# twosigma/Cook

Hardware: NVIDIA H100
Metric: job x offer fit evals/sec per scheduling cycle (higher is better)
Workload: dtype f64

## Files before the change

cook_b200/csrc/match.cu:

```cuda
#include <cooperative_groups.h>

#include <algorithm>
#include <mutex>
#include <numeric>

#include "fold.cuh"
#include "sort.cuh"

namespace {

constexpr int RES_THREADS = 512;
constexpr int TOPK = 8;
constexpr int ROW_V_OFF = TOPK * 32 * 8;
constexpr int ROW_BYTES = TOPK * 32 * (8 + 4);

struct __align__(32) VmStatic { double lc, lm, rc, rm; };
struct __align__(32) VmDyn { double ac, am, yc, ym; };
struct __align__(8) VmCnt { int an, pu; };

struct __align__(16) VmCons {
  int hostname_id, location, max_tasks, num_tasks;
  int run_count, flags, gpu_lo, ports_total;
  long long host_start;
  int disk_lo, disk_n;
// ... 514 lines not shown
              int tv = vv[i]; vv[i] = vv[i - 1]; vv[i - 1] = tv;
            }
          }
        }
      }
    }
  }
  const bool wany = __any_sync(0xffffffffu, f[0] > 0.0);
  if (wany) {
#pragma unroll
    for (int i = 0; i < TOPK; i++) { E.f[warp][i][lane] = f[i]; E.v[warp][i][lane] = vv[i]; }
  }
  if (lane == 0) E.any[warp] = wany ? 1 : 0;
  long long e1 = PROF ? clock64() : 0;
  __syncthreads();
  if (CONSTR && sparse)
    for (int wd = threadIdx.x; wd < a.sb_words; wd += NW * 32) __stcg(sbrow + wd, SP.sb[wd]);
  bool any = false;
#pragma unroll
  for (int w = 0; w < NW; w++) any |= E.any[w] != 0;
  if (any) {
    constexpr int PER = NW * TOPK / 32;
    static_assert(NW * TOPK % 32 == 0 && TOPK % PER == 0, "partial lists split evenly over the lanes");
#pragma unroll 1
    for (int ci = 0; ci < CPW; ci++) {
      const int c = warp + ci * NW;
      const int sw = lane / (TOPK / PER), so = (lane % (TOPK / PER)) * PER;
      double lf[PER];
      int lv[PER];
#pragma unroll
      for (int j = 0; j < PER; j++) {
        const bool has = E.any[sw] != 0;
        lf[j] = has ? E.f[sw][so + j][c] : 0.0;
        lv[j] = has ? E.v[sw][so + j][c] : 0x7fffffff;
      }
      double of = 0.0;
      int ov = -1;
#pragma unroll 1
      for (int i = 0; i < TOPK; i++) {
        unsigned wk;
        int wl;
        const double wf = warp_argmax(lf[0], (unsigned)lv[0], wk, wl);
        if (!(wf > 0.0)) break;
        if (lane == i) { of = wf; ov = (int)wk; }
        if (lane == wl) {
#pragma unroll
          for (int q = 0; q < PER - 1; q++) { lf[q] = lf[q + 1]; lv[q] = lv[q + 1]; }
          lf[PER - 1] = 0.0; lv[PER - 1] = 0x7fffffff;
        }
      }
      if (lane < TOPK) {
        __stcg(rf + lane * 32 + c, of);
        __stcg(rv + lane * 32 + c, ov);
      }
    }
  }
  long long e2 = PROF ? clock64() : 0;
  __syncthreads();
  if (threadIdx.x == 0) {
    if (any) atomicMax(a.feas + (size_t)(blk & 1) * a.bmax + ib, blk + 1);
    asm volatile("red.release.gpu.global.add.u32 [%0], %1;" ::"l"(a.rows_ready + blk), "r"(1u) : "memory");
  }
  if (PROF) {
    long long e3 = clock64();
    ep[0] += (unsigned long long)(e1 - e0); ep[1] += (unsigned long long)(e2 - e1);
    ep[2] += (unsigned long long)(e3 - e2);
  }
}

constexpr int MAXB = 512;
constexpr int LOGN = 2 * MAXB;
constexpr int RING = 32;
constexpr int GRING = 64;
constexpr int MAX_SPEC_CTAS = 8;
constexpr int KC = 16;
#ifndef COOK_LK
#define COOK_LK 4
#endif
constexpr int LK = COOK_LK;
#ifndef COOK_NCW
#define COOK_NCW 4
#endif
constexpr int NCW = COOK_NCW;

enum { Q_JOB = 0, Q_END = 1, Q_EXIT = 2 };

struct Latest {
  int* s;
  int* g;
  __device__ __forceinline__ int get(int v) const { return g ? g[v] : s[v]; }
  __device__ __forceinline__ void set(int v, int e) const { if (g) g[v] = e; else s[v] = e; }
};

__device__ __forceinline__ void fence_cta() { asm volatile("fence.acq_rel.cta;" ::: "memory"); }
__device__ __forceinline__ void compiler_barrier() { asm volatile("" ::: "memory"); }

struct QEntry {
  int type, blk, k, lo;
  double jc, jm, jg;
  int jports, jj, grp, row;
};

struct __align__(16) LogEnt {
  int vm, an, pu, k;
  double ac, am, lc, lm, rc, rm, yc, ym;
};

struct Cand {
  double f;
  VmState st;
  int vm, e;
};

struct __align__(16) SpecOut {
  int type, s, n, complete;
  double zf;
  int gver, pad;
  int zv, z_real;
  Cand c[KC + 1];
};

static_assert(sizeof(SpecOut) % 16 == 0, "candidate sets travel with cp.async.bulk (16 B granules)");
static_assert(RING == 32, "the fetcher warp owns one result slot per lane");

struct ResolverShared {
  LogEnt log[LOGN];
  int4 logx[LOGN];
  QEntry q[RING];
  SpecOut res[RING + 1];
  unsigned long long res_bar[RING];
  volatile int q_seq[RING];
  volatile unsigned long long chain;
  volatile int exit_g;
  int ticket;
  volatile int lo_ring[4];
  volatile int bk_ring[8];
  volatile int bk_known;
  volatile int out_done, blk_c0, last_b;
};

__device__ __forceinline__ int chain_gdone(unsigned long long w) { return (int)(w >> 32); }
__device__ __forceinline__ int chain_ncommit(unsigned long long w) { return (int)(unsigned)w; }
__device__ __forceinline__ unsigned long long chain_pack(int gdone, int ncommit) {
  return ((unsigned long long)(unsigned)gdone << 32) | (unsigned)ncommit;
}

template <bool CONSTR>
__device__ __forceinline__ VmState load_log(const ResolverShared& S, int idx, int& vm, int& k) {
  const LogEnt* e = &S.log[idx & (LOGN - 1)];
  const int4 h = *reinterpret_cast<const int4*>(e);
  const double2 a0 = *reinterpret_cast<const double2*>(&e->ac);
  const double2 a1 = *reinterpret_cast<const double2*>(&e->lc);
  const double2 a2 = *reinterpret_cast<const double2*>(&e->rc);
  const double2 a3 = *reinterpret_cast<const double2*>(&e->yc);
  VmState st;
  vm = h.x; st.an = h.y; st.pu = h.z; k = h.w;
  st.ac = a0.x; st.am = a0.y; st.lc = a1.x; st.lm = a1.y; st.rc = a2.x; st.rm = a2.y; st.yc = a3.x; st.ym = a3.y;
  st.room = 0x7fffffff; st.occ = 0; st.ptot = 0;
  if (CONSTR) {
    const int4 x = S.logx[idx & (LOGN - 1)];
    st.room = x.x; st.occ = x.y; st.ptot = x.z;
  }
  return st;
}
template <bool CONSTR>
__device__ __forceinline__ void store_log(ResolverShared& S, int idx, int vm, int k, const VmState& st) {
  LogEnt* e = &S.log[idx & (LOGN - 1)];
  *reinterpret_cast<int4*>(e) = make_int4(vm, st.an, st.pu, k);
  *reinterpret_cast<double2*>(&e->ac) = make_double2(st.ac, st.am);
  *reinterpret_cast<double2*>(&e->lc) = make_double2(st.lc, st.lm);
  *reinterpret_cast<double2*>(&e->rc) = make_double2(st.rc, st.rm);
  *reinterpret_cast<double2*>(&e->yc) = make_double2(st.yc, st.ym);
  if (CONSTR) S.logx[idx & (LOGN - 1)] = make_int4(st.room, st.occ, st.ptot, 0);
}

struct LaneList {
  double f[LK];
  int v[LK], e[LK];
  double cbf, dbf;
  int cbv, dbv;
  bool cb_real;
  __device__ __forceinline__ void init() {
#pragma unroll
    for (int i = 0; i < LK; i++) { f[i] = 0.0; v[i] = 0x7fffffff; e[i] = -1; }
    cbf = dbf = 0.0; cbv = dbv = 0x7fffffff; cb_real = false;
  }
  __device__ __forceinline__ void push_front(double x, int xv, int xe) {
#pragma unroll
    for (int i = LK - 1; i > 0; i--) { f[i] = f[i - 1]; v[i] = v[i - 1]; e[i] = e[i - 1]; }
    f[0] = x; v[0] = xv; e[0] = xe;
  }
  __device__ __forceinline__ void insert(double x, int xv, int xe) {
    if (!(x > 0.0)) return;
    if (!better(x, xv, f[LK - 1], v[LK - 1])) {
      if (better(x, xv, dbf, dbv)) { dbf = x; dbv = xv; }
      return;
    }
    if (f[LK - 1] > 0.0 && better(f[LK - 1], v[LK - 1], dbf, dbv)) { dbf = f[LK - 1]; dbv = v[LK - 1]; }
    f[LK - 1] = x; v[LK - 1] = xv; e[LK - 1] = xe;
#pragma unroll
    for (int i = LK - 1; i > 0; i--) {
      if (better(f[i], v[i], f[i - 1], v[i - 1])) {
        double tf = f[i]; f[i] = f[i - 1]; f[i - 1] = tf;
        int tv = v[i]; v[i] = v[i - 1]; v[i - 1] = tv;
        int te = e[i]; e[i] = e[i - 1]; e[i - 1] = te;
      }
    }
  }
};


__device__ __forceinline__ int group_version(const MatchArgs& a, int j) {
  int v = 0;
  for (int q = a.jb.group_off[j]; q < a.jb.group_off[j + 1]; q++) v += __ldcg(a.gr.gp_n + a.jb.group_idx[q]);
  return v;
}

template <bool CONSTR>
__device__ __forceinline__ void spec_job(const MatchArgs& a, ResolverShared& S, const Latest latest, const QEntry& qe,
                                         const int s, const int depth, const int exact_n, SpecOut& out) {
  const int lane = threadIdx.x & 31;
// ... 81 lines not shown
    int cnt = __popc(q);
    if (cnt > depth - n) {
      unsigned wk;
      int wl;
      warp_argmax(qual ? hf : 0.0, (unsigned)hv, wk, wl);
      q = 1u << wl;
      cnt = 1;
    }
    if ((q >> lane) & 1u) {
      store_cand(n + __popc(q & ((1u << lane) - 1u)), hf, hv, he);
      taken |= 1u << hj;
    }
    n += cnt;
  }
  double zf;
  int zv, z_real = 0;
  {
    double ef = 0.0;
    int ev = 0x7fffffff, ee = -1;
    bool head = false;
#pragma unroll
    for (int j = LK - 1; j >= 0; j--)
      if (L.f[j] > 0.0 && !((taken >> j) & 1u)) { ef = L.f[j]; ev = L.v[j]; ee = L.e[j]; head = true; }
    if (L.cbf > 0.0 && better(L.cbf, L.cbv, ef, ev)) { ef = L.cbf; ev = L.cbv; head = false; }
    if (L.dbf > 0.0 && better(L.dbf, L.dbv, ef, ev)) { ef = L.dbf; ev = L.dbv; head = false; }
    zf = warp_max_f64(ef);
    zv = (int)__reduce_min_sync(0xffffffffu, (ef == zf && zf > 0.0) ? (unsigned)ev : 0xffffffffu);
    if (!(zf > 0.0)) complete = 1;
    else {
      const unsigned hm = __ballot_sync(0xffffffffu, ef == zf && ev == zv);
      const unsigned rm = __ballot_sync(0xffffffffu, ef == zf && ev == zv && head);
      if (hm == rm && hm != 0u) {
        z_real = 1;
        if (lane == __ffs(rm) - 1) store_cand(KC, zf, zv, ee);
      }
    }
  }
  if (lane == 0) { out.type = Q_JOB; out.s = s; out.n = n; out.complete = complete; out.zf = zf; out.zv = zv; out.z_real = z_real; out.gver = gver; }
  __syncwarp();
}

template <bool CONSTR>
__device__ __noinline__ void spec_job_fallback(const MatchArgs& a, ResolverShared& S, const Latest latest,
                                               const QEntry& qe, const int s) {
  spec_job<CONSTR>(a, S, latest, qe, s, 1, 1, S.res[RING]);
}

template <bool CONSTR>
__device__ __noinline__ int resolve_group_job(const MatchArgs& a, ResolverShared& S, const Latest latest,
                                              const QEntry& qe, VmState& w) {
  const int lane = threadIdx.x & 31;
  JobRegs r;
  r.c = qe.jc; r.m = qe.jm; r.g = qe.jg; r.ports = qe.jports; r.j = qe.jj;
  const unsigned* sbrow = CONSTR ? a.sbits + ((size_t)(qe.blk & 1) * a.bmax + qe.row) * a.sb_words : nullptr;
  double cf = 0.0;
  int cv = 0x7fffffff;
  for (int v = lane; v < a.of.O; v += 32) {
    const int e = latest.get(v);
    VmState st;
    if (e >= qe.lo) { int vm, k; st = load_log<CONSTR>(S, e, vm, k); }
    else st = load_snap<CONSTR>(a, qe.blk, v);
    const double f = eval_res<CONSTR>(a, r, v, st, true, CONSTR ? sb_global(sbrow, v) : true);
    if (f > cf) { cf = f; cv = v; }
  }
  unsigned wk;
  int wl;
  const double wf = warp_argmax(cf, (unsigned)cv, wk, wl);
  if (!(wf > 0.0)) return -1;
  const int wv = (int)wk;
  const int we = latest.get(wv);
  if (we >= qe.lo) { int vm, k; w = load_log<CONSTR>(S, we, vm, k); }
  else w = load_snap<CONSTR>(a, qe.blk, wv);
  return wv;
}

template <bool CONSTR, bool REMOTE>
__device__ void driver_warp(const MatchArgs& a, ResolverShared& S) {
  const int lane = threadIdx.x & 31;
  int g = 0;
  unsigned long long skipped = 0;
  auto wait_slot = [&](int gi) {
    while (chain_gdone(S.chain) <= gi - a.lookahead) __nanosleep(a.poll_ns);
  };
  for (int b = 0;; b++) {
    int k0, k1;
    if (!REMOTE) {
      while (S.bk_known < b + 1) __nanosleep(20);
      k0 = S.bk_ring[b & 7];
      k1 = S.bk_ring[(b + 1) & 7];
    } else {
      if (b >= 2) {
        if (lane == 0) {
          while ((int)ld_relaxed_u32(a.published) < b - 1) __nanosleep(64);
          __threadfence();
        }
        __syncwarp();
      }
      k0 = __ldcg(a.bk0 + b);
      k1 = __ldcg(a.bk0 + b + 1);
    }
    if (k0 >= a.n_cons) break;
    const int nj = min(k1, a.n_cons) - k0;
    int dead = 0;
    if (lane == 0) {
      while (ld_acquire_u32(a.rows_ready + b) < (unsigned)nj) {
        const int db = (int)ld_relaxed_u32(reinterpret_cast<const unsigned*>(a.dead_blk));
        if (db != 0 && db - 1 <= b) { dead = 1; break; }
        __nanosleep(20);
      }
    }
    dead = __shfl_sync(0xffffffffu, dead, 0);
    if (dead) {
      if (!REMOTE && lane == 0) {
        skipped += (unsigned long long)(a.n_cons - k0);
        *a.dead_k0 = k0;
      }
      break;
    }
    const int lo = b == 0 ? 0 : (REMOTE ? __ldcg(a.lo_g + b - 1) : S.lo_ring[(b - 1) & 3]);
    const int32_t* feas = a.feas + (size_t)(b & 1) * a.bmax;
    int stamp[MAXB / 32];
#pragma unroll
    for (int t = 0; t < MAXB / 32; t++) stamp[t] = (t * 32 + lane) < nj ? __ldcg(feas + t * 32 + lane) : 0;
#pragma unroll
    for (int t = 0; t < MAXB / 32; t++) {
      const int base = t * 32;
      if (base >= nj) break;
      const int i = base + lane;
      const bool valid = i < nj;
      const bool fz = valid && stamp[t] == b + 1;
      if (!REMOTE && valid && !fz) { a.assign[k0 + i] = -1; a.fail[k0 + i] = COOK_FAIL_RESOURCES; }
      const unsigned mask = __ballot_sync(0xffffffffu, fz);
      skipped += __popc(__ballot_sync(0xffffffffu, valid && !fz));
      if (fz) {
        const int gi = g + __popc(mask & ((1u << lane) - 1u));
        const int k = k0 + i;
        QEntry q;
        q.type = Q_JOB; q.blk = b; q.k = k; q.lo = lo;
        q.jc = a.kc[k]; q.jm = a.km[k]; q.jj = a.cons[k];
        q.jg = CONSTR ? a.kg[k] : 0.0;
        q.jports = CONSTR ? a.kports[k] : 0;
        q.grp = CONSTR ? (a.kflags[k] & 1) : 0;
        q.row = i;
        wait_slot(gi);
        S.q[gi & (RING - 1)] = q;
        fence_cta();
        S.q_seq[gi & (RING - 1)] = gi + 1;
      }
      g += __popc(mask);
      __syncwarp();
    }
    if (lane == 0) {
      wait_slot(g);
      QEntry& q = S.q[g & (RING - 1)];
      q.type = Q_END; q.blk = b; q.k = -1; q.lo = lo; q.grp = 0;
      if (!REMOTE) S.res[g & (RING - 1)].type = Q_END;
      fence_cta();
      S.q_seq[g & (RING - 1)] = g + 1;
      if (!REMOTE) mbar_arrive(&S.res_bar[g & (RING - 1)]);
    }
    g++;
    __syncwarp();
  }
  if (lane == 0) {
    wait_slot(g);
    S.q[g & (RING - 1)].type = Q_EXIT;
    if (!REMOTE) S.res[g & (RING - 1)].type = Q_EXIT;
    fence_cta();
    S.q_seq[g & (RING - 1)] = g + 1;
    if (!REMOTE) mbar_arrive(&S.res_bar[g & (RING - 1)]);
    S.exit_g = g;
    if (!REMOTE) a.stats[6] = skipped;
  }
}

template <bool CONSTR>
__device__ void spec_warp(const MatchArgs& a, ResolverShared& S, const Latest latest, const int ci) {
  const int lane = threadIdx.x & 31;
  while (true) {
    int t = 0;
    if (lane == 0) t = atomicAdd(&S.ticket, 1);
    t = __shfl_sync(0xffffffffu, t, 0);
    const int g = t * a.n_spec + ci;
    const int slot = g & (RING - 1);
    bool quit = false;
    while (S.q_seq[slot] != g + 1) {
      const int xg = S.exit_g;
      if (xg >= 0 && g > xg) { quit = true; break; }
      __nanosleep(a.poll_ns);
    }
    if (quit) return;
    compiler_barrier();
    const QEntry qe = S.q[slot];
    if (qe.type == Q_EXIT) return;
    if (qe.type != Q_JOB) continue;
    const int s = chain_ncommit(S.chain);
    compiler_barrier();
    spec_job<CONSTR>(a, S, latest, qe, s, KC, 2, a.gres[g & (GRING - 1)]);
    __threadfence();
    __syncwarp();
    if (lane == 0) st_release_u32(a.gres_seq + (g & (GRING - 1)), (unsigned)(g + 1));
  }
}

template <bool CONSTR>
__device__ void publisher_warp(const MatchArgs& a, ResolverShared& S) {
  const int lane = threadIdx.x & 31;
  int p = 0;
  unsigned long long last = 0ull;
  while (true) {
    const unsigned long long w = S.chain;
    compiler_barrier();
    if (w != last) {
      const int c = chain_ncommit(w);
      for (int base = p; base < c; base += 6) {
        const int e = base + lane / 5, ch = lane % 5;
        if (lane < 30 && e < c) {
          const int4 v = reinterpret_cast<const int4*>(&S.log[e & (LOGN - 1)])[ch];
          __stcg(reinterpret_cast<int4*>(a.glog + (e & (LOGN - 1))) + ch, v);
        }
      }
      if (CONSTR)
        for (int e = p + lane; e < c; e += 32) __stcg(a.glogx + (e & (LOGN - 1)), S.logx[e & (LOGN - 1)]);
      __threadfence();
      __syncwarp();
      if (lane == 0) st_release_u64(a.gchain, w);
      p = c;
      last = w;
    } else {
      __nanosleep(40);
    }
    const int xg = S.exit_g;
    if (xg >= 0 && chain_gdone(last) >= xg) return;
  }
}

template <bool CONSTR>
__device__ void follower_warp(const MatchArgs& a, ResolverShared& S, const Latest latest) {
  const int lane = threadIdx.x & 31;
  int p = 0;
  unsigned long long last = 0ull;
  while (true) {
    unsigned long long w = 0ull;
    if (lane == 0) w = ld_relaxed_u64(a.gchain);
    w = __shfl_sync(0xffffffffu, w, 0);
    if (w != last) {
      __threadfence();
      const int c = chain_ncommit(w);
      for (int base = p; base < c; base += 6) {
        const int e = base + lane / 5, ch = lane % 5;
// ... 2 lines not shown
          reinterpret_cast<int4*>(&S.log[e & (LOGN - 1)])[ch] = v;
        }
      }
      if (CONSTR)
        for (int e = p + lane; e < c; e += 32) S.logx[e & (LOGN - 1)] = __ldcg(a.glogx + (e & (LOGN - 1)));
      __syncwarp();
      if (lane == 0) {
        for (int e = p; e < c; e++) latest.set(S.log[e & (LOGN - 1)].vm, e);
        fence_cta();
        S.chain = w;
      }
      __syncwarp();
      p = c;
      last = w;
    } else {
      __nanosleep(40);
    }
    const int xg = S.exit_g;
    if (xg >= 0 && chain_gdone(last) >= xg) return;
  }
}

__device__ void fetcher_warp(const MatchArgs& a, ResolverShared& S) {
  const int lane = threadIdx.x & 31;
  int g = lane;
  bool have_q = false, done = false;
  while (true) {
    if (!done && !have_q) {
      if (S.q_seq[lane] == g + 1) {
        compiler_barrier();
        const int type = S.q[lane].type;
        if (type == Q_JOB) have_q = true;
        else if (type == Q_EXIT) done = true;
        else g += RING;
      } else {
        const int xg = S.exit_g;
        if (xg >= 0 && g > xg) done = true;
      }
    }
    bool issued = false;
    if (!done && have_q) {
      const int gi = g & (GRING - 1);
      if (ld_relaxed_u32(a.gres_seq + gi) == (unsigned)(g + 1)) {
        __threadfence();
        fence_proxy_async_global();
        mbar_arrive_expect_tx(&S.res_bar[lane], (unsigned)sizeof(SpecOut));
        bulk_g2s(&S.res[lane], a.gres + gi, (unsigned)sizeof(SpecOut), &S.res_bar[lane]);
        have_q = false;
        g += RING;
        issued = true;
      }
    }
    if (__all_sync(0xffffffffu, done)) return;
    if (!__any_sync(0xffffffffu, issued)) __nanosleep(a.poll_ns);
  }
}

__device__ __forceinline__ double warp_argmax_fast(double f, int v, int& wv, int& wl) {
  const unsigned hi = (unsigned)__double2hiint(f);
  const unsigned mh = __reduce_max_sync(0xffffffffu, hi);
  unsigned cand = __ballot_sync(0xffffffffu, hi == mh);
  if (mh == 0u) { wv = 0x7fffffff; wl = 0; return 0.0; }
  if (__popc(cand) > 1) {
    const unsigned lo = hi == mh ? (unsigned)__double2loint(f) : 0u;
    const unsigned ml = __reduce_max_sync(0xffffffffu, lo);
    cand = __ballot_sync(0xffffffffu, hi == mh && lo == ml);
    if (__popc(cand) > 1) {
      const unsigned key = ((cand >> (threadIdx.x & 31)) & 1u) ? (unsigned)v : 0xffffffffu;
      const unsigned mk = __reduce_min_sync(0xffffffffu, key);
      cand = __ballot_sync(0xffffffffu, key == mk);
    }
  }
  wl = __ffs(cand) - 1;
  wv = __shfl_sync(0xffffffffu, v, wl);
  return __shfl_sync(0xffffffffu, f, wl);
}

template <bool CONSTR, bool PROF>
__device__ void commit_warp(const MatchArgs& a, ResolverShared& S, const Latest latest, const int cw,
                            unsigned* sbw) {
  const int lane = threadIdx.x & 31;
  unsigned long long n_fast = 0, n_group = 0, n_matched = 0, n_fallback = 0, n_slow_turn = 0, n_ztake = 0, n_relook = 0;
  unsigned long long prof[6] = {0, 0, 0, 0, 0, 0};
  const long long t_start = clock64();
  for (int g = cw;; g += NCW) {
    const int slot = g & (RING - 1);
    long long t0 = PROF ? clock64() : 0;
    bool quit = false;
    while (!mbar_try_wait(&S.res_bar[slot], (unsigned)(g >> 5) & 1u, 2000u)) {
      const int xg = S.exit_g;
      if (xg >= 0 && g > xg) { quit = true; break; }
    }
    if (quit) break;
    const SpecOut* R = &S.res[slot];
    const int type = R->type;
    if (PROF) prof[0] += (unsigned long long)(clock64() - t0);
    if (type == Q_EXIT) {
      while (chain_gdone(S.chain) != g) __nanosleep(20);
      if (lane == 0) a.stats[14] = (unsigned long long)(clock64() - t_start);
      break;
    }
    if (type == Q_END) {
      unsigned long long w;
      while (chain_gdone(w = S.chain) != g) __nanosleep(20);
      compiler_barrier();
      long long t4 = PROF ? clock64() : 0;
      const int b = S.q[slot].blk, lo = S.q[slot].lo;
      const int c = chain_ncommit(w), out_done = S.out_done;
      VmDyn* pub = a.dyn.d[b & 1];
      for (int e = lo + lane; e < c; e += 32) {
        int vm, k;
        const VmState st = load_log<CONSTR>(S, e, vm, k);
        if (latest.get(vm) == e) {
          __stcg(reinterpret_cast<double2*>(pub + vm), make_double2(st.ac, st.am));
          if (CONSTR) __stcg(reinterpret_cast<int2*>(a.dyn.n[b & 1] + vm), make_int2(st.an, st.pu));
        }
        if (e >= out_done) {
          a.assign[k] = vm;
          a.fail[k] = COOK_FAIL_NONE;
          a.ports_start[k] = CONSTR ? st.pu - a.kports[k] : 0;
        }
      }
      __syncwarp();
      if (lane == 0) {
        S.out_done = c;
        S.lo_ring[(b + 1) & 3] = c;
        const int nb = S.bk_ring[(b + 1) & 7] - S.bk_ring[b & 7];
        const int placed = c - S.blk_c0;
        long long want = placed > 0 ? ((long long)a.btarget * nb + placed - 1) / placed : a.bmax;
        want = min(want, (long long)min(a.bmax, 2 * S.last_b));
        const int nbn = max((int)want, a.bmin);
        S.last_b = nbn;
        S.blk_c0 = c;
        const int end2 = S.bk_ring[(b + 2) & 7] + nbn;
        S.bk_ring[(b + 3) & 7] = end2;
        __stcg(a.bk0 + b + 3, end2);
        __stcg(a.lo_g + b + 1, c);
        fence_cta();
        S.bk_known = b + 3;
        __threadfence();
        asm volatile("st.release.gpu.global.u32 [%0], %1;" ::"l"(a.published), "r"((unsigned)(b + 1)) : "memory");
        S.chain = chain_pack(g + 1, c);
        if (PROF && S.bk_ring[b & 7] < a.n_cons / 4) a.stats[15] = (unsigned long long)(clock64() - t_start);
      }
      __syncwarp();
      if (PROF) prof[4] += (unsigned long long)(clock64() - t4);
      continue;
    }
    const QEntry& qe = S.q[slot];
    JobRegs r;
    r.c = qe.jc; r.m = qe.jm; r.g = CONSTR ? qe.jg : 0.0; r.ports = CONSTR ? qe.jports : 0; r.j = qe.jj;
    const int k = qe.k;
    const bool grp = CONSTR && qe.grp;
    if (CONSTR) {
      const unsigned* sbrow = a.sbits + ((size_t)(qe.blk & 1) * a.bmax + qe.row) * a.sb_words;
      for (int wd = lane; wd < a.sb_words; wd += 32) sbw[wd] = __ldcg(sbrow + wd);
      __syncwarp();
    }
    auto join_groups = [&](int wv) {
      for (int q = a.jb.group_off[r.j]; q < a.jb.group_off[r.j + 1]; q++) {
        const int gi = a.jb.group_idx[q];
        const int n = __ldcg(a.gr.gp_n + gi);
        __stcg(a.gr.gp_vm + a.gr.gp_off[gi] + n, wv);
        __threadfence();
        __stcg(a.gr.gp_n + gi, n + 1);
      }
      __threadfence();
    };
    const int s = R->s, n = R->n;
    const bool r_complete = R->complete != 0;
    const double r_zf = R->zf;
    const int r_zv = R->zv;
    const int el = s + lane;
    const double yf = lane < n ? R->c[lane & (KC - 1)].f : 0.0;
    const int yv = lane < n ? R->c[lane & (KC - 1)].vm : 0x7fffffff;
    static_assert(KC <= 32 && (KC & (KC - 1)) == 0, "one candidate per lane");
    constexpr int TD = 3;
    double tf[TD];
    int tv[TD], ts[TD], d = 0;
#pragma unroll
    for (int i = 0; i < TD; i++) { tf[i] = 0.0; tv[i] = 0x7fffffff; ts[i] = 0; }
    bool more = false, have = false;
    int c_seen = s;
    long long t1 = PROF ? clock64() : 0;
    unsigned long long w;
    int c = 0;
  relook:
    while (true) {
      w = S.chain;
      compiler_barrier();
      const int gd = chain_gdone(w);
      const int c_now = chain_ncommit(w);
      const bool mine = gd == g;
      if (!have) {
        double xf = 0.0;
        int x_vm = 0x7fffffff;
        if (el < c_now) {
          int kk;
          const VmState x = load_log<CONSTR>(S, el, x_vm, kk);
          xf = eval_res<CONSTR>(a, r, x_vm, x, grp, CONSTR ? sb_shared(sbw, x_vm) : true);
        }
        c_seen = c_now;
        bool xin = el < c_seen && xf > 0.0 && latest.get(x_vm) == el;
        bool ok = lane < n && latest.get(yv) < s;
        const int nvalid = __popc(__ballot_sync(0xffffffffu, xin)) + __popc(__ballot_sync(0xffffffffu, ok));
        more = nvalid > TD;
        d = min(nvalid, TD);
#pragma unroll
        for (int rnd = 0; rnd < TD; rnd++) {
          const bool use_y = ok && (!xin || better(yf, yv, xf, x_vm));
          const double lf = use_y ? yf : (xin ? xf : 0.0);
          const int lv = use_y ? yv : (xin ? x_vm : 0x7fffffff);
          int bv, bl;
          const double bf = warp_argmax_fast(lf, lv, bv, bl);
          const bool by = __shfl_sync(0xffffffffu, use_y ? 1 : 0, bl) != 0;
          tf[rnd] = bf; tv[rnd] = bv; ts[rnd] = by ? ~bl : s + bl;
          if (lane == bl) { if (use_y) ok = false; else xin = false; }
        }
        have = true;
        if (mine) n_slow_turn++;
        continue;
      }
      if (mine && c_now <= c_seen + 1) { c = c_now; break; }
      if (c_now > c_seen) {
        int nvm, kk;
        const VmState ne = load_log<CONSTR>(S, c_seen, nvm, kk);
// ... 37 lines not shown
    int ne_vm = -1;
    double nf = 0.0;
    if (c > c_seen) {
      int kk;
      ne = load_log<CONSTR>(S, c_seen, ne_vm, kk);
      nf = eval_res<CONSTR>(a, r, ne_vm, ne, grp, CONSTR ? sb_shared(sbw, ne_vm) : true);
    }
    const bool first = !(d > 0 && tv[0] == ne_vm);
    const bool known = first ? (d > 0 || !more) : (d > 1 || !more);
    if (!known) {
      have = false;
      n_relook++;
      goto relook;
    }
    const double pf = first ? (d > 0 ? tf[0] : 0.0) : (d > 1 ? tf[1] : 0.0);
    const int pv = first ? (d > 0 ? tv[0] : 0x7fffffff) : (d > 1 ? tv[1] : 0x7fffffff);
    const int ps = first ? ts[0] : ts[1];
    const bool take_new = nf > 0.0 && better(nf, ne_vm, pf, pv);
    const double wf = take_new ? nf : pf;
    const int wv0 = take_new ? ne_vm : pv;
    const bool exact = known && (r_complete || (wf > 0.0 && better(wf, wv0, r_zf, r_zv)));
    const bool take_z = !exact && known && R->z_real != 0 && ne_vm != r_zv && latest.get(r_zv) < s;
    int wv = -1;
    auto append = [&](int vm, VmState st) {
      st.ac = st.ac + r.c; st.am = st.am + r.m; st.an += 1; st.pu += r.ports;
      store_log<CONSTR>(S, c, vm, k, st);
      latest.set(vm, c);
      if (grp) join_groups(vm);
      fence_cta();
      S.chain = chain_pack(g + 1, c + 1);
    };
    if (grp && group_version(a, r.j) != R->gver) {
      const QEntry q2 = qe;
      VmState ws;
      wv = resolve_group_job<CONSTR>(a, S, latest, q2, ws);
      n_group++;
      if (lane == 0) {
        if (wv >= 0) append(wv, ws);
        else S.chain = chain_pack(g + 1, c);
      }
    } else if (take_z) {
      n_fast++;
      n_ztake++;
      wv = r_zv;
      if (lane == 0) append(wv, R->c[KC].st);
    } else if (exact) {
      n_fast++;
      if (wf > 0.0) {
        wv = wv0;
        if (!take_new) {
          int vm2, kk;
          if (ps >= 0) ne = load_log<CONSTR>(S, ps, vm2, kk);
          else ne = R->c[(~ps) & (KC - 1)].st;
        }
        if (lane == 0) append(wv, ne);
      } else if (lane == 0) {
        S.chain = chain_pack(g + 1, c);
      }
    } else {
      const QEntry q2 = qe;
      const long long tf0 = PROF ? clock64() : 0;
      spec_job_fallback<CONSTR>(a, S, latest, q2, c);
      if (PROF) prof[5] += (unsigned long long)(clock64() - tf0);
      n_fallback++;
      const bool got = S.res[RING].n > 0;
      if (lane == 0) {
        if (got) append(S.res[RING].c[0].vm, S.res[RING].c[0].st);
        else S.chain = chain_pack(g + 1, c);
      }
      if (got) wv = 0;
    }
    if (wv >= 0) n_matched++;
    __syncwarp();
    if (PROF) prof[2] += (unsigned long long)(clock64() - t2);
  }
  if (lane == 0) {
    atomicAdd(a.stats + 0, n_fast); atomicAdd(a.stats + 2, n_group); atomicAdd(a.stats + 3, n_matched);
    atomicAdd(a.stats + 4, n_fallback); atomicAdd(a.stats + 7, n_slow_turn); atomicAdd(a.stats + 24, n_ztake); atomicAdd(a.stats + 25, n_relook);
    for (int i = 0; i < 6; i++) atomicAdd(a.stats + 8 + i, prof[i]);
  }
}

template <bool CONSTR, bool PROF>
__global__ void __launch_bounds__(RES_THREADS, 1) match_kernel(MatchArgs a) {
  extern __shared__ __align__(128) unsigned char smem_raw[];
  const int ns = a.n_spec;
  if ((int)blockIdx.x <= ns) {
    ResolverShared& S = *reinterpret_cast<ResolverShared*>(smem_raw);
    Latest latest;
    const size_t res_base = (sizeof(ResolverShared) + 15) & ~size_t(15);
    unsigned* sbw_base = reinterpret_cast<unsigned*>(smem_raw + res_base);
    latest.s = reinterpret_cast<int*>(smem_raw + res_base + (((size_t)NCW * a.sb_words * 4 + 15) & ~size_t(15)));
    latest.g = a.latest_global ? a.latest_global + (size_t)blockIdx.x * (size_t)(a.of.O + 1) : nullptr;
    const int warp = threadIdx.x >> 5;
    for (int i = threadIdx.x; i < a.of.O; i += RES_THREADS) latest.set(i, -1);
    if (threadIdx.x < RING) S.q_seq[threadIdx.x] = 0;
    for (int i = threadIdx.x; i < LOGN; i += RES_THREADS) S.log[i].vm = 0;
    if (threadIdx.x == 0) {
      S.chain = 0ull; S.exit_g = -1; S.ticket = 0;
      S.lo_ring[0] = S.lo_ring[1] = S.lo_ring[2] = S.lo_ring[3] = 0;
      S.bk_ring[0] = 0; S.bk_ring[1] = a.B; S.bk_ring[2] = 2 * a.B; S.bk_known = 2;
      S.out_done = 0; S.blk_c0 = 0; S.last_b = a.B;
      for (int i = 0; i < RING; i++) mbar_init(&S.res_bar[i], 1u);
      fence_proxy_async_smem();
    }
    __syncthreads();
    if (blockIdx.x == 0) {
      if (warp < NCW) commit_warp<CONSTR, PROF>(a, S, latest, warp, sbw_base + (size_t)warp * a.sb_words);
      else if (warp == NCW) driver_warp<CONSTR, false>(a, S);
      else if (warp == NCW + 1) publisher_warp<CONSTR>(a, S);
      else if (warp == NCW + 2) fetcher_warp(a, S);
    } else {
      if (warp == 0) follower_warp<CONSTR>(a, S, latest);
      else if (warp == 1) driver_warp<CONSTR, true>(a, S);
      else if (warp < a.max_spec_warp) spec_warp<CONSTR>(a, S, latest, (int)blockIdx.x - 1);
    }
  } else {
    EvalStatic es;
    es.lc = es.lm = es.rc = es.rm = nullptr;
    EvalShared& E = *reinterpret_cast<EvalShared*>(smem_raw);
    if (a.vs_in_smem) {
      double* base = reinterpret_cast<double*>(smem_raw + ((sizeof(EvalShared) + 127) & ~size_t(127)));
      const size_t O = (size_t)a.of.O;
      double* lc = base; double* lm = base + O; double* rc = base + 2 * O; double* rm = base + 3 * O;
      for (int v = threadIdx.x; v < a.of.O; v += RES_THREADS) {
        const VmStatic x = a.of.vs[v];
        lc[v] = x.lc; lm[v] = x.lm; rc[v] = x.rc; rm[v] = x.rm;
      }
      __syncthreads();
      es.lc = lc; es.lm = lm; es.rc = rc; es.rm = rm;
    }
    __shared__ int bk_s[2];
    __shared__ double smin_s[2];
    __shared__ double red_c[NW], red_m[NW];
    SparseLive& SP = *reinterpret_cast<SparseLive*>(
        smem_raw + ((sizeof(EvalShared) + 127) & ~size_t(127)) + (a.vs_in_smem ? (size_t)a.of.O * 32 : 0));
    if ((threadIdx.x >> 5) >= NW) return;
    const int n_eval = gridDim.x - 1 - ns;
    const int ei = (int)blockIdx.x - 1 - ns;
    unsigned long long work = 0, wait = 0, work_q1 = 0, rows_q1 = 0, nblk_seen = 0, n_hopeless = 0;
    unsigned long long ep[3] = {0, 0, 0};
    double capc = 0.0, capm = 0.0;
    {
      const double2* stb = reinterpret_cast<const double2*>(a.of.vs);
      for (int v = threadIdx.x; v < a.of.O; v += NW * 32) {
        double lc, lm;
        if (es.lc) { lc = es.lc[v]; lm = es.lm[v]; }
        else { const double2 s0 = __ldg(stb + 2 * v); lc = s0.x; lm = s0.y; }
        capc = fmax(capc, lc); capm = fmax(capm, lm);
      }
      for (int o = 16; o > 0; o >>= 1) { capc = fmax(capc, __shfl_xor_sync(0xffffffffu, capc, o)); capm = fmax(capm, __shfl_xor_sync(0xffffffffu, capm, o)); }
      if ((threadIdx.x & 31) == 0) { red_c[threadIdx.x >> 5] = capc; red_m[threadIdx.x >> 5] = capm; }
      __syncthreads();
      for (int w = 0; w < NW; w++) { capc = fmax(capc, red_c[w]); capm = fmax(capm, red_m[w]); }
      __syncthreads();
    }
    for (int b = 0;; b++) {
      long long w0 = clock64();
      if (threadIdx.x == 0) {
        if (b >= 2) {
          while ((int)ld_relaxed_u32(a.published) < b - 1) __nanosleep(32);
          __threadfence();
        }
        bk_s[0] = __ldcg(a.bk0 + b);
        bk_s[1] = __ldcg(a.bk0 + b + 1);
        if (bk_s[0] < a.n_cons) { smin_s[0] = a.smin_c[bk_s[0]]; smin_s[1] = a.smin_m[bk_s[0]]; }
      }
      __syncthreads();
      const int k0 = bk_s[0];
      const int k1 = min(bk_s[1], a.n_cons);
      const double minc = smin_s[0], minm = smin_s[1];
      __syncthreads();
      if (k0 >= a.n_cons) break;
      long long w1 = clock64();
      unsigned long long live = ~0ull;
      double maxfc = 1.7976931348623157e308, maxfm = 1.7976931348623157e308;
      if (a.of.O <= 64 * 32 * NW) {
        live = 0ull;
        double fc = -1.0, fm = -1.0;
        const double2* dyb = reinterpret_cast<const double2*>(a.dyn.d[b & 1]);
        const double2* stb = reinterpret_cast<const double2*>(a.of.vs);
        int u = 0;
        for (int v = 32 * (threadIdx.x >> 5) + (threadIdx.x & 31); v < a.of.O; v += 32 * NW, u++) {
          const double2 d0 = __ldcg(dyb + 2 * v);
          double lc, lm;
          if (es.lc) { lc = es.lc[v]; lm = es.lm[v]; }
          else { const double2 s0 = __ldg(stb + 2 * v); lc = s0.x; lm = s0.y; }
          bool dead = (d0.x + minc > lc) | (d0.y + minm > lm);
          bool special = false;
          if (CONSTR) {
            const int4* vcp = reinterpret_cast<const int4*>(a.of.vc + v);
            const int4 c0 = __ldg(vcp), c1 = __ldg(vcp + 1);
            const int an = __ldcg(reinterpret_cast<const int*>(a.dyn.n[b & 1] + v));
            if (c0.z >= 0 && !(c0.w + an < c0.z)) dead = true;
// ... 830 lines not shown
  CK(pool, csort::sort_indices(mp->d_pos, mp->d_tmp, n_ranked, LessUserPos{ca.ranked, ca.jb.user}, st));
  launches++;
  for (long long w = csort::TILE; w < n_ranked; w <<= 1) launches++;
  seg_bounds_kernel<<<(n_ranked + TB - 1) / TB, TB, 0, st>>>(SortedKey{mp->d_pos, ca.ranked, ca.jb.user}, n_ranked,
                                                             mp->d_seg_s, mp->d_seg_e, nullptr);
  CK(pool, cudaMemsetAsync(mp->d_gf, 0, sizeof(GridFlag), st));
  grid_check_kernel<<<(mp->J + TB - 1) / TB, TB, 0, st>>>(ca.jb.cpus, ca.jb.mem, ca.jb.gpus, mp->J, mp->d_gf);
  cons_user_kernel<<<(U + 3) / 4, 128, 0, st>>>(ca, mp->d_pos, mp->d_seg_s, mp->d_seg_e, mp->d_keep, mp->d_gf);
  launches++;
  const ConsOut cons_out{mp->d_cons, mp->d_kc, mp->d_km, mp->d_kg, mp->d_kports, mp->d_kflags};
  if (ca.pool_q.enabled) {
    cons_queue_kernel<<<1, 32, 0, st>>>(ca, mp->d_keep, cons_out, mp->d_counters);
    launches += 3;
  } else {
    compact(ConsSurvivors{ca, mp->d_keep, cons_out}, n_ranked, nullptr, mp->d_tmp, mp->d_counters, ca.num_considerable, st);
    launches += 5;
  }
  CK(pool, cudaGetLastError());
  int32_t n_cons = 0;
  CK(pool, cudaMemcpyAsync(&n_cons, mp->d_counters, sizeof(int32_t), cudaMemcpyDeviceToHost, st));
  CK(pool, cudaEventRecord(pool->ev[2], st));
  CK(pool, cudaStreamSynchronize(st));

  ma.n_cons = n_cons;
  int n_used = 0;
  unsigned long long hstats[32] = {0};
  const bool prof_on = getenv("COOK_PROF") != nullptr;
  CK(pool, cudaEventRecord(pool->ev[5], st));
  if (n_cons > 0) {
    if (O == 0) {
      CK(pool, cudaMemsetAsync(ma.assign, 0xff, sizeof(int32_t) * n_cons, st));
      CK(pool, cudaMemsetAsync(ma.fail, COOK_FAIL_NO_OFFERS, n_cons, st));
    } else {
      {
        const int nsb = (n_cons + SMIN_TB - 1) / SMIN_TB;
        suffix_min_local_kernel<<<nsb, SMIN_TB, 0, st>>>(mp->d_kc, mp->d_km, n_cons, mp->d_smin_c, mp->d_smin_m,
                                                         mp->d_smin_bc, mp->d_smin_bm);
        suffix_min_apply_kernel<<<nsb, SMIN_TB, 0, st>>>(n_cons, nsb, mp->d_smin_c, mp->d_smin_m, mp->d_smin_bc,
                                                         mp->d_smin_bm);
        launches += 2;
      }
      CK(pool, cudaMemsetAsync(ma.assign, 0xff, sizeof(int32_t) * n_cons, st));
      CK(pool, cudaMemsetAsync(ma.fail, COOK_FAIL_CONSTRAINT, n_cons, st));
      ma.sb_words = mp->constr ? (O + 31) / 32 : 0;
      const size_t res_base = ((sizeof(ResolverShared) + 15) & ~size_t(15)) +
                              (((size_t)NCW * ma.sb_words * 4 + 15) & ~size_t(15));
      size_t smem = res_base;
      ma.latest_global = nullptr;
      if (res_base + sizeof(int) * (size_t)O <= 200 * 1024) smem = std::max(smem, res_base + sizeof(int) * (size_t)O);
      else ma.latest_global = mp->d_latest;
      const size_t ev_base = (sizeof(EvalShared) + 127) & ~size_t(127);
      ma.vs_in_smem = ev_base + (size_t)O * 32 + sizeof(SparseLive) <= 224 * 1024 ? 1 : 0;
      if (getenv("COOK_NO_SMEM_STATIC")) ma.vs_in_smem = 0;
      ma.sparse_ok = getenv("COOK_NO_SPARSE") ? 0 : 1;
      smem = std::max(smem, ev_base + (ma.vs_in_smem ? (size_t)O * 32 : 0) + sizeof(SparseLive));
      void* kfn = mp->constr ? (prof_on ? (void*)match_kernel<true, true> : (void*)match_kernel<true, false>)
                             : (prof_on ? (void*)match_kernel<false, true> : (void*)match_kernel<false, false>);
      {
        static std::mutex mu;
        static int cur[16][4] = {};
        std::lock_guard<std::mutex> lk(mu);
        const int vi = (mp->constr ? 2 : 0) + (prof_on ? 1 : 0), di = pool->device & 15;
        if ((int)smem > cur[di][vi]) {
          int optin = 0;
          CK(pool, cudaDeviceGetAttribute(&optin, cudaDevAttrMaxSharedMemoryPerBlockOptin, pool->device));
          cudaFuncAttributes fa;
          CK(pool, cudaFuncGetAttributes(&fa, kfn));
          optin -= (int)fa.sharedSizeBytes;
          const int want = std::max((int)smem, optin);
          CK(pool, cudaFuncSetAttribute(kfn, cudaFuncAttributeMaxDynamicSharedMemorySize, std::min(want, optin)));
          cur[di][vi] = std::min(want, optin);
        }
        if ((int)smem > cur[di][vi])
          return set_err(pool, COOK_E_TOO_LARGE,
                         "cook_match: the offer table does not fit the kernel's shared memory (constraint pools: the verdict-bit "
                         "rows of the four owners bound a pool at about 130k offers) - split the pool");
      }
      int grid = pool->sm_count;
      if (max_ctas > 0) grid = std::min(grid, max_ctas);
      int occ = 0;
      CK(pool, cudaOccupancyMaxActiveBlocksPerMultiprocessor(&occ, kfn, RES_THREADS, smem));
      if (occ < 1) return set_err(pool, COOK_E_CUDA, "cook_match: kernel does not fit on an SM");
      if (grid < 3) grid = 3;
      int n_spec = 3;
      if (const char* es = getenv("COOK_NSPEC")) n_spec = atoi(es);
      n_spec = std::max(1, std::min(n_spec, std::min(MAX_SPEC_CTAS, std::max(1, grid / 8))));
      n_spec = std::min(n_spec, grid - 2);
      ma.n_spec = n_spec;
      void* kargs[] = {&ma};
      CK(pool, cudaLaunchCooperativeKernel(kfn, dim3(grid), dim3(RES_THREADS), kargs, smem, st));
      launches++;
    }
  }
  CK(pool, cudaEventRecord(pool->ev[6], st));
  if (n_cons > 0) {
    finalize_kernel<<<(n_cons + TB - 1) / TB, TB, 0, st>>>(ma, mp->d_out_assign,
                                                           out_ports ? mp->d_out_ports : nullptr,
                                                           max_ports, mp->d_used);
    count_flags_kernel<<<(O + TB) / TB, TB, 0, st>>>(mp->d_used, O, mp->d_counters + 1);
    launches += 2;
    CK(pool, cudaGetLastError());
  }
  CK(pool, cudaEventRecord(pool->ev[3], st));
  if (n_cons > 0) {
    CK(pool, cudaMemcpyAsync(out_considerable, mp->d_cons, sizeof(int32_t) * n_cons, cudaMemcpyDeviceToHost, st));
    CK(pool, cudaMemcpyAsync(out_assign, mp->d_out_assign, sizeof(int32_t) * n_cons, cudaMemcpyDeviceToHost, st));
    if (out_ports && max_ports > 0)
      CK(pool, cudaMemcpyAsync(out_ports, mp->d_out_ports, sizeof(int32_t) * (size_t)n_cons * max_ports,
                               cudaMemcpyDeviceToHost, st));
    if (out_fail_reason)
      CK(pool, cudaMemcpyAsync(out_fail_reason, ma.fail, n_cons, cudaMemcpyDeviceToHost, st));
    CK(pool, cudaMemcpyAsync(hstats, mp->d_stats, sizeof(hstats), cudaMemcpyDeviceToHost, st));
    CK(pool, cudaMemcpyAsync(&n_used, mp->d_counters + 1, sizeof(int32_t), cudaMemcpyDeviceToHost, st));
  }
  CK(pool, cudaEventRecord(pool->ev[4], st));
  CK(pool, cudaStreamSynchronize(st));
  if (prof_on) {
    const char* nm[27] = {"fast", "chunk_rescan", "group_jobs", "matched", "fallbacks", "trunc_specs",
                          "skipped", "slow_turns", "c_wait_result", "c_follow_log", "c_decide_commit", "c_to_argmax",
                          "c_end_block", "c_fallback", "res_total", "res_q1_done", "eval_work", "eval_wait",
                          "eval_loop", "eval_sync", "eval_merge", "eval_work_q1", "eval_rowslots_q1", "blocks", "z_takes", "relooks", "rows_pretest_ei0"};
    for (int i = 0; i < 27; i++) fprintf(stderr, "[cook_prof] %-14s %llu\n", nm[i], hstats[i]);
  }
  mp->last_n_cons = n_cons;
  {
    cook_phase_stats& ps = pool->phase[COOK_PHASE_MATCH];
    ps.ms_h2d = uploaded ? ev_ms(pool->ev[0], pool->ev[1]) : 0.0;
    ps.ms_device = ev_ms(pool->ev[1], pool->ev[3]);
    ps.ms_d2h = ev_ms(pool->ev[3], pool->ev[4]);
    ps.h2d_bytes = uploaded ? mp->h2d_bytes : 0;
    ps.d2h_bytes = (int64_t)n_cons * (8 + (out_fail_reason ? 1 : 0) + (out_ports ? 4 * (int64_t)max_ports : 0)) + 44;
    ps.n_launches = launches;
  }
  if (out_stats) {
    out_stats->n_considerable = n_cons;
    out_stats->n_matched = (int)hstats[3];
    out_stats->head_matched = (n_cons > 0 && out_assign[0] >= 0) ? 1 : 0;
    out_stats->n_offers_used = n_used;
    out_stats->evals = (int64_t)n_cons * O;
    out_stats->n_fast = (int64_t)(hstats[0] + hstats[6]);
    out_stats->n_chunk_rescan = (int64_t)(hstats[1] + hstats[4]);
    out_stats->n_full_rescan = (int64_t)hstats[2];
    out_stats->ms_h2d = uploaded ? ev_ms(pool->ev[0], pool->ev[1]) : 0.0;
    out_stats->ms_considerable = ev_ms(pool->ev[1], pool->ev[2]);
    out_stats->ms_match = ev_ms(pool->ev[2], pool->ev[3]);
    out_stats->ms_match_kernel = ev_ms(pool->ev[5], pool->ev[6]);
    out_stats->ms_d2h = ev_ms(pool->ev[3], pool->ev[4]);
    out_stats->n_launches = launches;
    out_stats->h2d_bytes = uploaded ? mp->h2d_bytes : 0;
    out_stats->d2h_bytes = (int64_t)n_cons * (8 + (out_fail_reason ? 1 : 0) +
                                               (out_ports ? 4 * (int64_t)max_ports : 0)) + 44;
  }
  return COOK_OK;
}

extern "C" int32_t cook_match(cook_pool* pool, const int32_t* ranked_idx, int32_t n_ranked,
                              const cook_jobs_soa* jobs, const cook_offers_soa* offers,
                              const cook_groups* groups, const cook_user_table* users,
                              const cook_pool_quota* pool_quota, const cook_match_params* params,
                              int32_t* out_considerable, int32_t* out_assign, int32_t* out_ports,
                              int32_t max_ports, uint8_t* out_fail_reason,
                              cook_match_stats* out_stats) {
  if (!pool) return COOK_E_BADARG;
  if (!ranked_idx || !jobs || !offers || !users || !params || !out_considerable || !out_assign)
    return set_err(pool, COOK_E_BADARG, "cook_match: null argument");
  if (params->good_enough_fitness < 1.0)
    return set_err(pool, COOK_E_BADARG,
                   "cook_match: good_enough_fitness < 1.0 is Fenzo's racy early-exit mode; "
                   "only the deterministic mode (>= 1.0) is supported");
  if (params->fitness_kind != 0)
    return set_err(pool, COOK_E_UNSUPPORTED_CONSTRAINT, "cook_match: only cpuMemBinPacker");
  const int J = jobs->n, O = offers->n, U = users->n_users;
  const int NC = params->num_considerable;
  if (J < 0 || O < 0 || U <= 0 || n_ranked < 0 || NC < 0 || max_ports < 0)
    return set_err(pool, COOK_E_BADARG, "cook_match: bad sizes");
  if (out_stats) memset(out_stats, 0, sizeof(*out_stats));
  if (n_ranked == 0 || NC == 0) return COOK_OK;
  if (!params->reuse_resident) {
    if (!idx_in_range(ranked_idx, n_ranked, 0, J)) return set_err(pool, COOK_E_BADARG, "cook_match: ranked_idx out of range");
    if (!idx_in_range(jobs->user, J, 0, U)) return set_err(pool, COOK_E_BADARG, "cook_match: jobs.user out of range");
    if (jobs->attr_off && !idx_in_range(jobs->attr_col, jobs->attr_off[J], 0, std::max(1, offers->n_attr_cols)))
      return set_err(pool, COOK_E_BADARG, "cook_match: jobs.attr_col out of range");
    if (!offers->name_rank && O > 0) return set_err(pool, COOK_E_BADARG, "cook_match: offers.name_rank required");
    if (groups && !idx_in_range(groups->attr_col, groups->n_groups, -1, std::max(1, offers->n_attr_cols)))
      return set_err(pool, COOK_E_BADARG, "cook_match: groups.attr_col out of range");
  }
  CK(pool, cudaSetDevice(pool->device));
  if (!pool->match_plan) {
    pool->match_plan = new MatchPlan();
    pool->match_plan_free = plan_free;
  }
  MatchPlan* mp = static_cast<MatchPlan*>(pool->match_plan);
  const bool reuse = params->reuse_resident && mp->valid && mp->J == J && mp->O == O && mp->U == U &&
                     mp->n_ranked == n_ranked && mp->NC == NC && mp->max_ports == max_ports;
  if (params->reuse_resident && !reuse)
    return set_err(pool, COOK_E_BADARG,
                   "cook_match: reuse_resident set but no matching resident inputs on this handle");
  CK(pool, cudaEventRecord(pool->ev[0], pool->stream));
  if (!reuse) {
    int32_t rc = build_plan(pool, mp, ranked_idx, n_ranked, jobs, offers, groups, users, pool_quota,
                            params, max_ports);
    if (rc != COOK_OK) { mp->valid = false; return rc; }
  }
  return run_plan(pool, mp, out_considerable, out_assign, out_ports, out_fail_reason, out_stats, !reuse,
                  params->max_ctas);
// ... 109 lines not shown
```

Baseline: 27.70 billion.

## Move block-end publishing onto a dedicated warp overlapping the commit chain

Block-end work (publishing the newest VM state, writing assignments, sizing the next block and releasing the published flag) moves out of the commit warp and onto a new block-end warp. The commit chain can then advance to the next block without waiting for that publish loop. To stay correct, the driver waits when log-ring reuse would overwrite unpublished entries, and the publisher rescans the log when the latest index has moved past the block. It also raises the default speculative CTA count to 4 for unconstrained pools, and adds extra handshake state and a possible quadratic rescan in exchange.

After: 28.49 billion, median of 6. 2.9% higher.

```diff
diff --git a/cook_b200/csrc/match.cu b/cook_b200/csrc/match.cu
--- a/cook_b200/csrc/match.cu
+++ b/cook_b200/csrc/match.cu
@@ -620,6 +620,7 @@
 #define COOK_NCW 4
 #endif
 constexpr int NCW = COOK_NCW;
+static_assert(NCW + 4 <= RES_THREADS / 32, "the resolver CTA also runs a driver, publisher, fetcher and block-end warp");
 
 enum { Q_JOB = 0, Q_END = 1, Q_EXIT = 2 };
 
@@ -628,6 +629,9 @@
   int* g;
   __device__ __forceinline__ int get(int v) const { return g ? g[v] : s[v]; }
   __device__ __forceinline__ void set(int v, int e) const { if (g) g[v] = e; else s[v] = e; }
+  __device__ __forceinline__ int get_fresh(int v) const {
+    return g ? __ldcg(g + v) : *reinterpret_cast<const volatile int*>(s + v);
+  }
 };
 
 __device__ __forceinline__ void fence_cta() { asm volatile("fence.acq_rel.cta;" ::: "memory"); }
@@ -674,7 +678,7 @@
   volatile int lo_ring[4];
   volatile int bk_ring[8];
   volatile int bk_known;
-  volatile int out_done, blk_c0, last_b;
+  volatile int be_seq, be_done, be_lo, be_c, n_end;
 };
 
 __device__ __forceinline__ int chain_gdone(unsigned long long w) { return (int)(w >> 32); }
@@ -922,7 +926,9 @@
   auto wait_slot = [&](int gi) {
     while (chain_gdone(S.chain) <= gi - a.lookahead) __nanosleep(a.poll_ns);
   };
-  for (int b = 0;; b++) {
+  int lo_prev = 0, n_prev = 0;
+  int b = 0;
+  for (;; b++) {
     int k0, k1;
     if (!REMOTE) {
       while (S.bk_known < b + 1) __nanosleep(20);
@@ -959,6 +965,7 @@
     }
     const int lo = b == 0 ? 0 : (REMOTE ? __ldcg(a.lo_g + b - 1) : S.lo_ring[(b - 1) & 3]);
     const int32_t* feas = a.feas + (size_t)(b & 1) * a.bmax;
+    const int g0 = g;
     int stamp[MAXB / 32];
 #pragma unroll
     for (int t = 0; t < MAXB / 32; t++) stamp[t] = (t * 32 + lane) < nj ? __ldcg(feas + t * 32 + lane) : 0;
@@ -982,6 +989,8 @@
         q.jports = CONSTR ? a.kports[k] : 0;
         q.grp = CONSTR ? (a.kflags[k] & 1) : 0;
         q.row = i;
+        if (!REMOTE && lo + n_prev + (gi - g0) >= lo_prev + LOGN)
+          while (S.be_done < b) __nanosleep(a.poll_ns);
         wait_slot(gi);
         S.q[gi & (RING - 1)] = q;
         fence_cta();
@@ -990,6 +999,8 @@
       g += __popc(mask);
       __syncwarp();
     }
+    lo_prev = lo;
+    n_prev = g - g0;
     if (lane == 0) {
       wait_slot(g);
       QEntry& q = S.q[g & (RING - 1)];
@@ -1006,6 +1017,7 @@
     wait_slot(g);
     S.q[g & (RING - 1)].type = Q_EXIT;
     if (!REMOTE) S.res[g & (RING - 1)].type = Q_EXIT;
+    S.n_end = b;
     fence_cta();
     S.q_seq[g & (RING - 1)] = g + 1;
     if (!REMOTE) mbar_arrive(&S.res_bar[g & (RING - 1)]);
@@ -1174,7 +1186,6 @@
   const int lane = threadIdx.x & 31;
   unsigned long long n_fast = 0, n_group = 0, n_matched = 0, n_fallback = 0, n_slow_turn = 0, n_ztake = 0, n_relook = 0;
   unsigned long long prof[6] = {0, 0, 0, 0, 0, 0};
-  const long long t_start = clock64();
   for (int g = cw;; g += NCW) {
     const int slot = g & (RING - 1);
     long long t0 = PROF ? clock64() : 0;
@@ -1189,51 +1200,23 @@
     if (PROF) prof[0] += (unsigned long long)(clock64() - t0);
     if (type == Q_EXIT) {
       while (chain_gdone(S.chain) != g) __nanosleep(20);
-      if (lane == 0) a.stats[14] = (unsigned long long)(clock64() - t_start);
       break;
     }
     if (type == Q_END) {
+      const int b = S.q[slot].blk, lo = S.q[slot].lo;
       unsigned long long w;
       while (chain_gdone(w = S.chain) != g) __nanosleep(20);
       compiler_barrier();
       long long t4 = PROF ? clock64() : 0;
-      const int b = S.q[slot].blk, lo = S.q[slot].lo;
-      const int c = chain_ncommit(w), out_done = S.out_done;
-      VmDyn* pub = a.dyn.d[b & 1];
-      for (int e = lo + lane; e < c; e += 32) {
-        int vm, k;
-        const VmState st = load_log<CONSTR>(S, e, vm, k);
-        if (latest.get(vm) == e) {
-          __stcg(reinterpret_cast<double2*>(pub + vm), make_double2(st.ac, st.am));
-          if (CONSTR) __stcg(reinterpret_cast<int2*>(a.dyn.n[b & 1] + vm), make_int2(st.an, st.pu));
-        }
-        if (e >= out_done) {
-          a.assign[k] = vm;
-          a.fail[k] = COOK_FAIL_NONE;
-          a.ports_start[k] = CONSTR ? st.pu - a.kports[k] : 0;
-        }
-      }
-      __syncwarp();
       if (lane == 0) {
-        S.out_done = c;
+        const int c = chain_ncommit(w);
+        while (S.be_done < b) __nanosleep(20);
+        S.be_lo = lo;
+        S.be_c = c;
         S.lo_ring[(b + 1) & 3] = c;
-        const int nb = S.bk_ring[(b + 1) & 7] - S.bk_ring[b & 7];
-        const int placed = c - S.blk_c0;
-        long long want = placed > 0 ? ((long long)a.btarget * nb + placed - 1) / placed : a.bmax;
-        want = min(want, (long long)min(a.bmax, 2 * S.last_b));
-        const int nbn = max((int)want, a.bmin);
-        S.last_b = nbn;
-        S.blk_c0 = c;
-        const int end2 = S.bk_ring[(b + 2) & 7] + nbn;
-        S.bk_ring[(b + 3) & 7] = end2;
-        __stcg(a.bk0 + b + 3, end2);
-        __stcg(a.lo_g + b + 1, c);
         fence_cta();
-        S.bk_known = b + 3;
-        __threadfence();
-        asm volatile("st.release.gpu.global.u32 [%0], %1;" ::"l"(a.published), "r"((unsigned)(b + 1)) : "memory");
+        S.be_seq = b + 1;
         S.chain = chain_pack(g + 1, c);
-        if (PROF && S.bk_ring[b & 7] < a.n_cons / 4) a.stats[15] = (unsigned long long)(clock64() - t_start);
       }
       __syncwarp();
       if (PROF) prof[4] += (unsigned long long)(clock64() - t4);
@@ -1437,6 +1420,74 @@
 }
 
 template <bool CONSTR, bool PROF>
+__device__ void block_end_warp(const MatchArgs& a, ResolverShared& S, const Latest latest) {
+  const int lane = threadIdx.x & 31;
+  const long long t_start = clock64();
+  unsigned long long busy = 0;
+  int c_prev = 0, last_b = a.B;
+  for (int b = 0;; b++) {
+    bool quit = false;
+    while (S.be_seq <= b) {
+      if (S.exit_g >= 0) {
+        compiler_barrier();
+        if (S.n_end <= b) { quit = true; break; }
+      }
+      __nanosleep(40);
+    }
+    if (quit) break;
+    fence_cta();
+    const long long t0 = PROF ? clock64() : 0;
+    const int lo = S.be_lo, c = S.be_c;
+    VmDyn* pub = a.dyn.d[b & 1];
+    for (int e = lo + lane; e < c; e += 32) {
+      int vm, k;
+      const VmState st = load_log<CONSTR>(S, e, vm, k);
+      const int le = latest.get_fresh(vm);
+      bool newest = le == e;
+      if (le >= c) {
+        newest = true;
+        for (int x = e + 1; x < c && newest; x++) newest = S.log[x & (LOGN - 1)].vm != vm;
+      }
+      if (newest) {
+        __stcg(reinterpret_cast<double2*>(pub + vm), make_double2(st.ac, st.am));
+        if (CONSTR) __stcg(reinterpret_cast<int2*>(a.dyn.n[b & 1] + vm), make_int2(st.an, st.pu));
+      }
+      if (e >= c_prev) {
+        a.assign[k] = vm;
+        a.fail[k] = COOK_FAIL_NONE;
+        a.ports_start[k] = CONSTR ? st.pu - a.kports[k] : 0;
+      }
+    }
+    const int nb = S.bk_ring[(b + 1) & 7] - S.bk_ring[b & 7];
+    const int placed = c - c_prev;
+    long long want = placed > 0 ? ((long long)a.btarget * nb + placed - 1) / placed : a.bmax;
+    want = min(want, (long long)min(a.bmax, 2 * last_b));
+    const int nbn = max((int)want, a.bmin);
+    last_b = nbn;
+    __syncwarp();
+    if (lane == 0) {
+      const int end2 = S.bk_ring[(b + 2) & 7] + nbn;
+      S.bk_ring[(b + 3) & 7] = end2;
+      __stcg(a.bk0 + b + 3, end2);
+      __stcg(a.lo_g + b + 1, c);
+      fence_cta();
+      S.bk_known = b + 3;
+      __threadfence();
+      asm volatile("st.release.gpu.global.u32 [%0], %1;" ::"l"(a.published), "r"((unsigned)(b + 1)) : "memory");
+      S.be_done = b + 1;
+      if (PROF && S.bk_ring[b & 7] < a.n_cons / 4) a.stats[15] = (unsigned long long)(clock64() - t_start);
+    }
+    c_prev = c;
+    __syncwarp();
+    if (PROF) busy += (unsigned long long)(clock64() - t0);
+  }
+  if (lane == 0) {
+    a.stats[14] = (unsigned long long)(clock64() - t_start);
+    if (PROF) a.stats[27] = busy;
+  }
+}
+
+template <bool CONSTR, bool PROF>
 __global__ void __launch_bounds__(RES_THREADS, 1) match_kernel(MatchArgs a) {
   extern __shared__ __align__(128) unsigned char smem_raw[];
   const int ns = a.n_spec;
@@ -1455,7 +1506,7 @@
       S.chain = 0ull; S.exit_g = -1; S.ticket = 0;
       S.lo_ring[0] = S.lo_ring[1] = S.lo_ring[2] = S.lo_ring[3] = 0;
       S.bk_ring[0] = 0; S.bk_ring[1] = a.B; S.bk_ring[2] = 2 * a.B; S.bk_known = 2;
-      S.out_done = 0; S.blk_c0 = 0; S.last_b = a.B;
+      S.be_seq = 0; S.be_done = 0; S.be_lo = 0; S.be_c = 0; S.n_end = 0;
       for (int i = 0; i < RING; i++) mbar_init(&S.res_bar[i], 1u);
       fence_proxy_async_smem();
     }
@@ -1465,6 +1516,7 @@
       else if (warp == NCW) driver_warp<CONSTR, false>(a, S);
       else if (warp == NCW + 1) publisher_warp<CONSTR>(a, S);
       else if (warp == NCW + 2) fetcher_warp(a, S);
+      else if (warp == NCW + 3) block_end_warp<CONSTR, PROF>(a, S, latest);
     } else {
       if (warp == 0) follower_warp<CONSTR>(a, S, latest);
       else if (warp == 1) driver_warp<CONSTR, true>(a, S);
@@ -2461,7 +2513,7 @@
       CK(pool, cudaOccupancyMaxActiveBlocksPerMultiprocessor(&occ, kfn, RES_THREADS, smem));
       if (occ < 1) return set_err(pool, COOK_E_CUDA, "cook_match: kernel does not fit on an SM");
       if (grid < 3) grid = 3;
-      int n_spec = 3;
+      int n_spec = mp->constr ? 3 : 4;
       if (const char* es = getenv("COOK_NSPEC")) n_spec = atoi(es);
       n_spec = std::max(1, std::min(n_spec, std::min(MAX_SPEC_CTAS, std::max(1, grid / 8))));
       n_spec = std::min(n_spec, grid - 2);
@@ -2495,11 +2547,12 @@
   CK(pool, cudaEventRecord(pool->ev[4], st));
   CK(pool, cudaStreamSynchronize(st));
   if (prof_on) {
-    const char* nm[27] = {"fast", "chunk_rescan", "group_jobs", "matched", "fallbacks", "trunc_specs",
+    const char* nm[28] = {"fast", "chunk_rescan", "group_jobs", "matched", "fallbacks", "trunc_specs",
                           "skipped", "slow_turns", "c_wait_result", "c_follow_log", "c_decide_commit", "c_to_argmax",
                           "c_end_block", "c_fallback", "res_total", "res_q1_done", "eval_work", "eval_wait",
-                          "eval_loop", "eval_sync", "eval_merge", "eval_work_q1", "eval_rowslots_q1", "blocks", "z_takes", "relooks", "rows_pretest_ei0"};
-    for (int i = 0; i < 27; i++) fprintf(stderr, "[cook_prof] %-14s %llu\n", nm[i], hstats[i]);
+                          "eval_loop", "eval_sync", "eval_merge", "eval_work_q1", "eval_rowslots_q1", "blocks", "z_takes", "relooks", "rows_pretest_ei0",
+                          "be_publish"};
+    for (int i = 0; i < 28; i++) fprintf(stderr, "[cook_prof] %-14s %llu\n", nm[i], hstats[i]);
   }
   mp->last_n_cons = n_cons;
   {
```
